# matteo-bastico/MI-Seg

Measured on AMD Instinct MI355X. Metric: 96^3 patches/sec fwd+bwd, C-Swin-UNETR fs=48 6-class, higher is better.
Workload: dtype bf16; 1 GPU; configs[1]: C-Swin-UNETR feature_size=48 heads=(3,6,12,24) instance_cond, 96^3 patch, 6 classes, batch 1 per GPU, fwd+bwd (+ gradient all-reduce at N>1); global_batch=1

## Files before the change

include/miseg_hip.h:

```cpp
#ifndef MISEG_HIP_H
#define MISEG_HIP_H
#include <stddef.h>
#include <stdint.h>

#ifdef __cplusplus
extern "C" {
#endif

typedef void* miseg_stream_t;

enum { MISEG_F32 = 0, MISEG_BF16 = 1 };
enum { MISEG_OK = 0, MISEG_E_BADARG = -1, MISEG_E_UNSUPPORTED = -2, MISEG_E_LAUNCH = -3 };
enum { MISEG_ACT_NONE = 0, MISEG_ACT_LEAKY = 1, MISEG_ACT_GELU = 2, MISEG_ACT_PRELU = 3 };
#define MISEG_MAX_STYLES 4

#define MISEG_ABI_VERSION 16
int miseg_abi_version(void);
const char* miseg_last_error(void);
int miseg_device_arch(char* buf, size_t n);

size_t miseg_instnorm_stat_bytes(int B, int C);
typedef struct {
  const void* x; int64_t ldx;
  int B, S, C, dtype;
// ... 205 lines not shown
  int wd, wh, ww, sd, sh, sw, tw;
  float scale;
  float drop_p; uint64_t drop_seed, drop_stream; const uint64_t* drop_step_dev;
} miseg_winattn_params;
int miseg_winattn_fwd(const miseg_winattn_params* p, miseg_stream_t stream);
int miseg_winattn_on_matrix_cores(const miseg_winattn_params* p);

typedef struct {
  miseg_winattn_params f;
  const void* dout; int64_t lddo;
  void* dqkv; int64_t lddq;
  float* dqkv_bias;
  float* dbias_table;
} miseg_winattn_bwd_params;
int miseg_winattn_bwd(const miseg_winattn_bwd_params* p, miseg_stream_t stream);

typedef struct { const void* a; int64_t lda; const void* b; int64_t ldb; void* y; int64_t ldy; int64_t rows; int C, dtype; } miseg_add_params;
int miseg_add(const miseg_add_params* p, miseg_stream_t stream);
typedef struct { uint32_t struct_size; const void* a; int64_t lda; const void* x; int64_t ldx; void* y; int64_t ldy; const float* coef; int B, S, C, dtype; } miseg_affine2_params;
int miseg_affine2(const miseg_affine2_params* p, miseg_stream_t stream);

typedef struct { const void* src; int64_t lds; int sdtype; void* dst; int64_t ldd; int ddtype; int64_t rows; int C; } miseg_copy2d_params;
int miseg_copy2d(const miseg_copy2d_params* p, miseg_stream_t stream);

typedef struct { const float* src; void* dst; int R, C, dtype, transpose; } miseg_cast_params;
int miseg_cast_matrix(const miseg_cast_params* p, miseg_stream_t stream);

typedef struct {
  const float* src; void* dst;
  int32_t R, C, transpose, inner, outer, tile0;
// ... 222 lines not shown
```

include/miseg_hip_debug.h:

```cpp
#ifndef MISEG_HIP_DEBUG_H
#define MISEG_HIP_DEBUG_H
#include "miseg_hip.h"
#ifdef __cplusplus
extern "C" {
#endif

int miseg_flag_wait(const uint64_t* flag_dev, const uint64_t* want_dev, uint64_t timeout_us, uint32_t* timed_out_dev, miseg_stream_t stream);
int miseg_streams_run_concurrently(miseg_stream_t a, miseg_stream_t b);
int miseg_debug_stamp(uint64_t* slot_dev, miseg_stream_t stream);

int miseg_prof_arm(int tag);
int miseg_prof_read(int* tags, float* ms, int max);

typedef void* miseg_graph_split_t;
typedef struct {
  int nodes, lanes, segments, crossing_edges, side_streams, main_lane_nodes;
  int streams_concurrent;
} miseg_graph_split_info;
int miseg_graph_split_create(void* hip_graph, miseg_stream_t launch_stream, int max_side_streams, miseg_graph_split_t* out,
                             miseg_graph_split_info* info );
int miseg_graph_split_launch(miseg_graph_split_t plan, miseg_stream_t stream);
void miseg_graph_split_destroy(miseg_graph_split_t plan);

int miseg_prof_available(void);

#ifdef __cplusplus
}
#endif
#endif
```

mi-seg_amd/csrc/attention.hip:

```cpp
#include "common.h"

namespace miseg {

struct WinGeom {
  int B, D, H, W, C, heads, hd;
  int wd, wh, ww, sd, sh, sw, tw;
  int Dp, Hp, Wp, nwd, nwh, nww, n;
  float scale;
};

__device__ __forceinline__ void token_info(const WinGeom& g, int win, int t, int& row, int& label, int& code) {
  int wi = win;
  const int wx = wi % g.nww; wi /= g.nww;
  const int wy = wi % g.nwh; wi /= g.nwh;
  const int wz = wi % g.nwd;
  const int b = wi / g.nwd;
  const int tz = t / (g.wh * g.ww), ty = (t / g.ww) % g.wh, tx = t % g.ww;
  const int pz = wz * g.wd + tz, py = wy * g.wh + ty, px = wx * g.ww + tx;
  int z = pz + g.sd; if (z >= g.Dp) z -= g.Dp;
  int y = py + g.sh; if (y >= g.Hp) y -= g.Hp;
  int x = px + g.sw; if (x >= g.Wp) x -= g.Wp;
  row = (z < g.D && y < g.H && x < g.W) ? ((b * g.D + z) * g.H + y) * g.W + x : -1;
  const int rz = g.sd ? (pz < g.Dp - g.wd ? 0 : (pz < g.Dp - g.sd ? 1 : 2)) : 0;
  const int ry = g.sh ? (py < g.Hp - g.wh ? 0 : (py < g.Hp - g.sh ? 1 : 2)) : 0;
// ... 337 lines not shown
  }
  return f;
}

__device__ __forceinline__ void att_load16v(const bf16* p, bool vec, float* dst) {
  if (vec) {
    const bf16x8 a = *reinterpret_cast<const bf16x8*>(p), b = *reinterpret_cast<const bf16x8*>(p + 8);
#pragma unroll
    for (int d = 0; d < 8; ++d) { dst[d] = to_f32(a[d]); dst[8 + d] = to_f32(b[d]); }
  } else {
#pragma unroll
    for (int d = 0; d < 16; ++d) dst[d] = to_f32(p[d]);
  }
}

__device__ __forceinline__ void att_unit(int heads, int& win, int& head) {
  const int nb = gridDim.x, xcd = blockIdx.x & 7, q = nb >> 3, r = nb & 7;
  const int unit = xcd * q + (xcd < r ? xcd : r) + (blockIdx.x >> 3);
  win = unit / heads;
  head = unit - win * heads;
}

template <bool MASK, int NW = 4, bool DROP = false>
__global__ void __launch_bounds__(NW * 64) winattn_fwd_mfma_kernel(const bf16* __restrict__ qkv, int64_t ldq, bf16* __restrict__ out, int64_t ldo,
                                                               const float* __restrict__ qkv_bias, const float* __restrict__ bias_table,
                                                               float* __restrict__ lse_out, WinGeom g, int tsize, bool vec, AttnDrop dr) {
  extern __shared__ __attribute__((aligned(16))) char smem[];
  bf16* Qs = reinterpret_cast<bf16*>(smem);
  bf16* Ks = Qs + ATT_NP * 16;
  bf16* Vt = Ks + ATT_NP * 16;
  int* kofs = reinterpret_cast<int*>(Vt + 16 * ATT_VT_LD);
  int* klab = kofs + ATT_NP;
  int* rowq = klab + ATT_NP;
// ... 156 lines not shown
#pragma unroll
    for (int d = 0; d < 8; ++d) { dst[d] = to_f32(a[d]); dst[8 + d] = to_f32(b[d]); }
  } else {
#pragma unroll
    for (int d = 0; d < 16; ++d) dst[d] = to_f32(p[d]);
  }
}

typedef unsigned pk2 __attribute__((ext_vector_type(2)));
__device__ __forceinline__ unsigned att_pk_bf16(float a, float b) {
  typedef float f32x2_ __attribute__((ext_vector_type(2)));
  typedef __bf16 bf16x2_ __attribute__((ext_vector_type(2)));
  return __builtin_bit_cast(unsigned, __builtin_convertvector(f32x2_{a, b}, bf16x2_));
}

template <bool MASK, bool DT , int NW = 4, bool DROP = false>
__global__ void __launch_bounds__(NW * 64, 2) winattn_bwd_mfma_kernel(const bf16* __restrict__ qkv, int64_t ldq, const bf16* __restrict__ out, int64_t ldo,
                                                                  const bf16* __restrict__ dout, int64_t lddo, bf16* __restrict__ dqkv, int64_t lddq,
                                                                  const float* __restrict__ qkv_bias, const float* __restrict__ bias_table,
                                                                  const float* __restrict__ lse_in, float* __restrict__ dqkv_bias,
                                                                  float* __restrict__ dbias_table, WinGeom g, int tsize, bool vec, AttnDrop dr) {
  extern __shared__ __attribute__((aligned(16))) char smem[];
  constexpr int NI = 24 / NW, NTHR = NW * 64;
  float* table = reinterpret_cast<float*>(smem);
  int* dtable = reinterpret_cast<int*>(table + ATT_TMAX);
  float* padb = reinterpret_cast<float*>(dtable + ATT_TMAX);
  unsigned* bound = reinterpret_cast<unsigned*>(padb + 48);
  char* dstile = reinterpret_cast<char*>(padb + 64);
  float* dqpart = reinterpret_cast<float*>(dstile + NW * 16 * ATT_DS_LD);
  int* qcode = reinterpret_cast<int*>(dqpart + 2 * NW * 256);
  int* qlabel = qcode + ATT_NP;
  int* rowq = qlabel + ATT_NP;
  float* nlse = reinterpret_cast<float*>(rowq + ATT_NP);
  float* ndelta = nlse + ATT_NP;
  bf16* Qs = reinterpret_cast<bf16*>(ndelta + ATT_NP);
  bf16* Gs = Qs + ATT_NP * 16;
  bf16* Ks = Gs + ATT_NP * 16;
  int win, head;
  att_unit(g.heads, win, head);
  const int tid = threadIdx.x;
  const int n = g.n, C = g.C, nt16 = (n + 15) / 16;
  if (tid < 52) padb[tid] = 0.f;
  __syncthreads();
  float mg2 = 0.f, mv2 = 0.f, mda = 0.f;
  for (int t = tid; t < nt16 * 16; t += NTHR) {
    int row = -1, label = 0, code = 0;
    float q[16], k[16], go[16];
    float dl = 0.f, ls = INFINITY, g2 = 0.f, v2 = 0.f;
#pragma unroll
    for (int d = 0; d < 16; ++d) q[d] = k[d] = go[d] = 0.f;
    if (t < n) {
      token_info(g, win, t, row, label, code);
      ls = lse_in[((int64_t)win * g.heads + head) * n + t];
      float v[16];
      if (row >= 0) {
        float o[16];
        att_load16(qkv + (int64_t)row * ldq + head * 16, vec, q);
        att_load16(qkv + (int64_t)row * ldq + C + head * 16, vec, k);
        att_load16(qkv + (int64_t)row * ldq + 2 * C + head * 16, vec, v);
        att_load16(dout + (int64_t)row * lddo + head * 16, vec, go);
        att_load16(out + (int64_t)row * ldo + head * 16, vec, o);
#pragma unroll
        for (int d = 0; d < 16; ++d) { dl = fmaf(go[d], o[d], dl); g2 = fmaf(go[d], go[d], g2); }
      } else {
#pragma unroll
        for (int d = 0; d < 16; ++d) {
          q[d] = qkv_bias ? qkv_bias[head * 16 + d] : 0.f;
          k[d] = qkv_bias ? qkv_bias[C + head * 16 + d] : 0.f;
          v[d] = qkv_bias ? qkv_bias[2 * C + head * 16 + d] : 0.f;
        }
      }
#pragma unroll
      for (int d = 0; d < 16; ++d) v2 = fmaf(v[d], v[d], v2);
    }
    mg2 = fmaxf(mg2, g2); mv2 = fmaxf(mv2, v2); mda = fmaxf(mda, fabsf(dl));
    const float qs = g.scale * ATT_LOG2E;
#pragma unroll
    for (int d = 0; d < 16; ++d) q[d] *= qs;
    att_store_row(Qs, t, q);
    att_store_row(Ks, t, k);
    att_store_row(Gs, t, go);
    qcode[t] = code * 4;
    qlabel[t] = label;
    rowq[t] = row;
    nlse[t] = -ls * ATT_LOG2E;
    ndelta[t] = -dl;
  }
#pragma unroll
  for (int o2 = 1; o2 < 64; o2 <<= 1) { mg2 = fmaxf(mg2, __shfl_xor(mg2, o2, 64)); mv2 = fmaxf(mv2, __shfl_xor(mv2, o2, 64)); mda = fmaxf(mda, __shfl_xor(mda, o2, 64)); }
  if ((tid & 63) == 0) { atomicMax(&bound[0], __float_as_uint(mg2)); atomicMax(&bound[1], __float_as_uint(mv2)); atomicMax(&bound[2], __float_as_uint(mda)); }
  for (int i = tid; i < tsize; i += NTHR) { table[i] = bias_table[(int64_t)i * g.heads + head] * ATT_LOG2E; dtable[i] = 0; }
  __syncthreads();
  const float bmax = sqrtf(__uint_as_float(bound[0]) * __uint_as_float(bound[1])) + __uint_as_float(bound[2]);
  const float fscale = bmax > 0.f ? 536870912.f / ((float)(n > 256 ? n : 256) * bmax) : 0.f;
  const int lane = tid & 63, wave = __builtin_amdgcn_readfirstlane(tid >> 6), fi = lane & 15, kg = lane >> 4;
  const int tb = 2 * g.tw - 1;
  const int centre = ((g.tw - 1) * tb + (g.tw - 1)) * tb + (g.tw - 1);
  constexpr float MASKV = -100.f * ATT_LOG2E;

  s16x4 kfB[NI], vfB[NI], kA[NI];
  f32x4 dvt[NI], dkt[NI];
  int ck[NI], lk[NI];
  const char* tkb[NI];
  bool kval = true;
  int itail = -1;
#pragma unroll
  for (int i = 0; i < NI; ++i) {
    const int kt = wave + NW * i;
    dvt[i] = dkt[i] = f32x4{0.f, 0.f, 0.f, 0.f};
    kfB[i] = vfB[i] = kA[i] = s16x4{0, 0, 0, 0};
    ck[i] = lk[i] = 0;
    tkb[i] = reinterpret_cast<const char*>(table);
    if (kt < nt16) {
      const int ki = kt * 16 + fi;
      kfB[i] = att_ld4(Ks, ki, kg);
      kA[i] = att_tr_rows(Ks, kt * 16, fi, kg);
      ck[i] = qcode[ki] - 4 * centre;
      tkb[i] = reinterpret_cast<const char*>(table) - ck[i];
      lk[i] = qlabel[ki];
      float v[4] = {0.f, 0.f, 0.f, 0.f};
      if (ki < n) {
        const int row = rowq[ki];
        if (row >= 0) {
          const bf16x4 t4 = *reinterpret_cast<const bf16x4*>(qkv + (int64_t)row * ldq + 2 * C + head * 16 + 4 * kg);
#pragma unroll
          for (int e = 0; e < 4; ++e) v[e] = to_f32(t4[e]);
        } else if (qkv_bias) {
#pragma unroll
          for (int e = 0; e < 4; ++e) v[e] = qkv_bias[2 * C + head * 16 + 4 * kg + e];
        }
      }
      vfB[i] = __builtin_bit_cast(s16x4, bf16x4{(bf16)v[0], (bf16)v[1], (bf16)v[2], (bf16)v[3]});
      if (kt == nt16 - 1 && (n & 15)) { itail = i; kval = ki < n; }
    }
  }
  const uint64_t dk0 = DROP ? dropout_step_key(dr.key, dr.step_dev) : 0ull;
  const int dcg = (n + 3) / 4;
  const int64_t dbase = ((int64_t)win * g.heads + head) * n;
  char* mytile = dstile + wave * 16 * ATT_DS_LD;
  char* const ds_w = mytile + fi * ATT_DS_LD + kg * 8;
  const char* const ds_r = mytile + (4 * kg + (fi >> 2)) * ATT_DS_LD + (fi & 3) * 8;

  f32x4 padq = f32x4{0.f, 0.f, 0.f, 0.f};
  for (int qt = 0; qt < nt16; ++qt) {
    const int q0 = qt * 16;
    const int4 qc4 = *reinterpret_cast<const int4*>(qcode + q0 + 4 * kg);
    const int qc[4] = {qc4.x, qc4.y, qc4.z, qc4.w};
    int ql[4] = {0, 0, 0, 0};
    if (MASK) {
      const int4 ql4 = *reinterpret_cast<const int4*>(qlabel + q0 + 4 * kg);
      ql[0] = ql4.x; ql[1] = ql4.y; ql[2] = ql4.z; ql[3] = ql4.w;
    }
    const f32x4 nl4 = *reinterpret_cast<const f32x4*>(nlse + q0 + 4 * kg);
    const f32x4 nd4 = *reinterpret_cast<const f32x4*>(ndelta + q0 + 4 * kg);
    const s16x4 qfA = att_ld4(Qs, q0 + fi, kg);
    const s16x4 gfA = att_ld4(Gs, q0 + fi, kg);
    const s16x4 qtA = att_tr_rows(Qs, q0, fi, kg);
    const s16x4 gtA = att_tr_rows(Gs, q0, fi, kg);
    f32x4 dq = f32x4{0.f, 0.f, 0.f, 0.f};
#pragma unroll
    for (int i = 0; i < NI; ++i) {
      if (wave + NW * i < nt16) {
        const f32x4 sacc = __builtin_amdgcn_mfma_f32_16x16x16bf16_1k(qfA, kfB[i], nl4, 0, 0, 0);
        const f32x4 pacc = __builtin_amdgcn_mfma_f32_16x16x16bf16_1k(gfA, vfB[i], DROP ? f32x4{0.f, 0.f, 0.f, 0.f} : nd4, 0, 0, 0);
        float pv[4], dsv[4], tbv[4];
        int bidx[4];
#pragma unroll
        for (int e = 0; e < 4; ++e) {
          bidx[e] = qc[e] - ck[i];
          tbv[e] = *reinterpret_cast<const float*>(tkb[i] + qc[e]);
        }
#pragma unroll
        for (int e = 0; e < 4; ++e) {
          float sc = sacc[e] + tbv[e];
          if (MASK) sc += (ql[e] != lk[i]) ? MASKV : 0.f;
          pv[e] = __builtin_amdgcn_exp2f(sc);
        }
        if (i == itail) {
#pragma unroll
          for (int e = 0; e < 4; ++e) pv[e] = kval ? pv[e] : 0.f;
        }
        float pm[4];
        if (DROP) {
          const int ki = (wave + NW * i) * 16 + fi;
#pragma unroll
          for (int e = 0; e < 4; ++e) {
            const uint64_t hh = dropout_group_hash(dk0, dbase + q0 + 4 * kg + e, dcg, ki);
            pm[e] = dropout_keeps(hh, ki, dr.thresh) ? pv[e] * dr.scale : 0.f;
            dsv[e] = fmaf(pm[e], pacc[e], pv[e] * nd4[e]);
          }
        } else {
#pragma unroll
          for (int e = 0; e < 4; ++e) { pm[e] = pv[e]; dsv[e] = pv[e] * pacc[e]; }
        }
        const pk2 pbp = pk2{att_pk_bf16(pm[0], pm[1]), att_pk_bf16(pm[2], pm[3])};
        const pk2 dbp = pk2{att_pk_bf16(dsv[0], dsv[1]), att_pk_bf16(dsv[2], dsv[3])};
        const s16x4 pb = __builtin_bit_cast(s16x4, pbp), db = __builtin_bit_cast(s16x4, dbp);
        const bf16x4 db4 = __builtin_bit_cast(bf16x4, dbp);
        dvt[i] = __builtin_amdgcn_mfma_f32_16x16x16bf16_1k(gtA, pb, dvt[i], 0, 0, 0);
        dkt[i] = __builtin_amdgcn_mfma_f32_16x16x16bf16_1k(qtA, db, dkt[i], 0, 0, 0);
        *reinterpret_cast<bf16x4*>(ds_w) = db4;
        __builtin_amdgcn_fence(__ATOMIC_RELEASE, "wavefront");
        __builtin_amdgcn_wave_barrier();
        __builtin_amdgcn_fence(__ATOMIC_ACQUIRE, "wavefront");
        const s16x4 dsT = att_tr4(ds_r);
        dq = __builtin_amdgcn_mfma_f32_16x16x16bf16_1k(kA[i], dsT, dq, 0, 0, 0);
        __builtin_amdgcn_wave_barrier();
        if (DT) {
#pragma unroll
          for (int e = 0; e < 4; ++e)
            atomicAdd(reinterpret_cast<int*>(reinterpret_cast<char*>(dtable) + bidx[e]), __float_as_int(fmaf(dsv[e], fscale, 12582912.f)) - 0x4B400000);
        }
      }
    }
    float* part = dqpart + (qt & 1) * (NW * 256);
    *reinterpret_cast<f32x4*>(part + (wave * 16 + fi) * 16 + 4 * kg) = dq;
    __syncthreads();
    if (wave == (qt & (NW - 1))) {
      const int ql_ = lane >> 2, d4 = lane & 3, t = q0 + ql_;
      f32x4 sum = *reinterpret_cast<const f32x4*>(part + ql_ * 16 + 4 * d4);
#pragma unroll
      for (int w = 1; w < NW; ++w) sum += *reinterpret_cast<const f32x4*>(part + (w * 16 + ql_) * 16 + 4 * d4);
      if (t < n) {
        const int row = rowq[t];
        if (row >= 0) {
          *reinterpret_cast<bf16x4*>(dqkv + (int64_t)row * lddq + head * 16 + 4 * d4) =
              bf16x4{(bf16)(sum[0] * g.scale), (bf16)(sum[1] * g.scale), (bf16)(sum[2] * g.scale), (bf16)(sum[3] * g.scale)};
        } else if (dqkv_bias) {
          padq += sum;
        }
      }
    }
  }
  if (dqkv_bias) {
#pragma unroll
    for (int o2 = 4; o2 < 64; o2 <<= 1)
#pragma unroll
      for (int e = 0; e < 4; ++e) padq[e] += __shfl_xor(padq[e], o2, 64);
    if (lane < 4) {
#pragma unroll
      for (int e = 0; e < 4; ++e)
        if (padq[e] != 0.f) atomicAdd(&padb[4 * lane + e], padq[e] * g.scale);
    }
  }
  constexpr float LN2 = 0.6931471805599453f;
  f32x4 padk = f32x4{0.f, 0.f, 0.f, 0.f}, padv = f32x4{0.f, 0.f, 0.f, 0.f};
#pragma unroll
  for (int i = 0; i < NI; ++i) {
    const int ki = (wave + NW * i) * 16 + fi;
    if (wave + NW * i < nt16 && ki < n) {
      const int row = rowq[ki];
      if (row >= 0) {
        bf16* pk = dqkv + (int64_t)row * lddq + C + head * 16 + 4 * kg;
        *reinterpret_cast<bf16x4*>(pk) = bf16x4{(bf16)(dkt[i][0] * LN2), (bf16)(dkt[i][1] * LN2), (bf16)(dkt[i][2] * LN2), (bf16)(dkt[i][3] * LN2)};
        *reinterpret_cast<bf16x4*>(pk + C) = bf16x4{(bf16)dvt[i][0], (bf16)dvt[i][1], (bf16)dvt[i][2], (bf16)dvt[i][3]};
      } else if (dqkv_bias) {
        padk += dkt[i];
        padv += dvt[i];
      }
    }
  }
  if (dqkv_bias) {
#pragma unroll
    for (int o2 = 1; o2 < 16; o2 <<= 1)
#pragma unroll
      for (int e = 0; e < 4; ++e) { padk[e] += __shfl_xor(padk[e], o2, 64); padv[e] += __shfl_xor(padv[e], o2, 64); }
    if (fi == 0) {
#pragma unroll
      for (int e = 0; e < 4; ++e) {
        if (padk[e] != 0.f) atomicAdd(&padb[16 + 4 * kg + e], padk[e] * LN2);
        if (padv[e] != 0.f) atomicAdd(&padb[32 + 4 * kg + e], padv[e]);
      }
    }
  }
  __syncthreads();
  if (dbias_table)
    for (int i = tid; i < tsize; i += NTHR) {
      const int v = dtable[i];
      if (v != 0) atomicAdd(dbias_table + (int64_t)i * g.heads + head, (float)v / fscale);
    }
  if (dqkv_bias && tid < 48) {
    const float v = padb[tid];
    if (v != 0.f) atomicAdd(dqkv_bias + (tid >> 4) * C + head * 16 + (tid & 15), v);
  }
}

static size_t attn_mfma_bwd_smem(int tsize, int nw = 4) {
  (void)tsize;
  return (size_t)3 * ATT_NP * 32 + (size_t)5 * ATT_NP * 4 + (size_t)2 * nw * 256 * 4 + (size_t)nw * 16 * ATT_DS_LD + 64 * 4 + (size_t)2 * ATT_TMAX * 4;
}

static size_t attn_mfma_fwd_smem(int tsize) {
  return (size_t)(2 * ATT_NP * 16 + 16 * ATT_VT_LD) * 2 + (size_t)3 * ATT_NP * 4 + (size_t)tsize * 4;
}

int global_attn_fwd(const miseg_winattn_params* p, const AttnDrop& dr, hipStream_t s, int* rc);
int global_attn_bwd(const miseg_winattn_bwd_params* p, const AttnDrop& dr, hipStream_t s, int* rc);
bool global_attn_takes(const miseg_winattn_params* p);

// ... 79 lines not shown
#undef FWD_MFMA_D
    MISEG_LAUNCH_CHECK("winattn_fwd_mfma");
    return MISEG_OK;
  }
  return dispatch_dtype(p->dtype, [&](auto* tag) -> int {
    typedef typename std::remove_pointer<decltype(tag)>::type T;
    HD_SWITCH(g.hd / 4, {
      MISEG_SET_SMEM((winattn_fwd_kernel<T, HD4>), sh);
      winattn_fwd_kernel<T, HD4><<<grid, threads, sh, s>>>((const T*)p->qkv, p->ldq, (T*)p->out, p->ldo, p->qkv_bias, p->bias_table, p->lse, g, tsize, dr);
    });
    MISEG_LAUNCH_CHECK("winattn_fwd");
    return MISEG_OK;
  });
}

extern "C" int miseg_winattn_bwd(const miseg_winattn_bwd_params* p, miseg_stream_t s_) {
  hipStream_t s = (hipStream_t)s_;
  MISEG_REQUIRE(p && p->dout && p->dqkv, MISEG_E_BADARG, "winattn_bwd: null pointer");
  WinGeom g;
  int rc = make_geom(&p->f, &g);
  if (rc) return rc;
  MISEG_REQUIRE(p->f.drop_p >= 0.f && p->f.drop_p < 1.f, MISEG_E_BADARG, "winattn_bwd: drop_p = %f must lie in [0, 1)", (double)p->f.drop_p);
  const AttnDrop dr = attn_drop_args(&p->f);
  if (global_attn_bwd(p, dr, s, &rc)) return rc;
  const int tb = 2 * g.tw - 1, tsize = p->f.bias_table ? tb * tb * tb : 0;
  const size_t sh = attn_smem_bytes(g.n, g.hd, tsize, true);
  MISEG_REQUIRE(sh <= 160 * 1024, MISEG_E_UNSUPPORTED, "winattn_bwd: %zu bytes of LDS needed", sh);
  dim3 grid(g.B * g.nwd * g.nwh * g.nww, g.heads);
  const int threads = cdiv(g.n, 64) * 64;
  if (p->f.dtype == MISEG_BF16 && g.hd == 16 && g.n <= ATT_NP && p->f.bias_table && tsize <= ATT_TMAX && ((uintptr_t)p->dqkv % 8 == 0) && p->lddq % 4 == 0 &&
      ((uintptr_t)p->f.qkv % 8 == 0) && p->f.ldq % 4 == 0) {
    const bool vec = p->f.ldq % 8 == 0 && p->f.ldo % 8 == 0 && p->lddo % 8 == 0 && (uintptr_t)p->f.qkv % 16 == 0 && (uintptr_t)p->f.out % 16 == 0 &&
                     (uintptr_t)p->dout % 16 == 0;
    const bool wide = true;
    const size_t shm = attn_mfma_bwd_smem(tsize, wide ? 8 : 4);
#define BWD_MFMA_X(M, D, NWV, X)                                                                                                                            \
  MISEG_SET_SMEM((winattn_bwd_mfma_kernel<M, D, NWV, X>), shm);                              \
  winattn_bwd_mfma_kernel<M, D, NWV, X><<<grid.x * grid.y, NWV * 64, shm, s>>>((const bf16*)p->f.qkv, p->f.ldq, (const bf16*)p->f.out, p->f.ldo, (const bf16*)p->dout,    \
                                                                    p->lddo, (bf16*)p->dqkv, p->lddq, p->f.qkv_bias, p->f.bias_table, p->f.lse, p->dqkv_bias, \
                                                                    p->dbias_table, g, tsize, vec, dr)
#define BWD_MFMA(M, D, NWV) do { if (dr.thresh) { BWD_MFMA_X(M, D, NWV, true); } else { BWD_MFMA_X(M, D, NWV, false); } } while (0)
#define BWD_MFMA_W(M, D) do { if (wide) { BWD_MFMA(M, D, 8); } else { BWD_MFMA(M, D, 4); } } while (0)
    const bool masked = (g.sd | g.sh | g.sw) != 0;
    if (p->dbias_table) { if (masked) BWD_MFMA_W(true, true); else BWD_MFMA_W(false, true); }
    else { if (masked) BWD_MFMA_W(true, false); else BWD_MFMA_W(false, false); }
#undef BWD_MFMA_W
#undef BWD_MFMA
#undef BWD_MFMA_X
    MISEG_LAUNCH_CHECK("winattn_bwd_mfma");
    return MISEG_OK;
  }
  return dispatch_dtype(p->f.dtype, [&](auto* tag) -> int {
    typedef typename std::remove_pointer<decltype(tag)>::type T;
    HD_SWITCH(g.hd / 4, {
      MISEG_SET_SMEM((winattn_bwd_kernel<T, HD4>), sh);
      winattn_bwd_kernel<T, HD4><<<grid, threads, sh, s>>>((const T*)p->f.qkv, p->f.ldq, (const T*)p->f.out, p->f.ldo, (const T*)p->dout, p->lddo, (T*)p->dqkv, p->lddq,
                                                           p->f.qkv_bias, p->f.bias_table, p->f.lse, p->dqkv_bias, p->dbias_table ? p->dbias_table : nullptr, g,
                                                           tsize, dr);
    });
    MISEG_LAUNCH_CHECK("winattn_bwd");
// ... 4 lines not shown
```

mi-seg_amd/hip/lib.py:

```python
import ctypes as C
import os

HERE = os.path.dirname(os.path.abspath(__file__))
LIB_PATH = os.environ.get("MISEG_HIP_LIB") or os.path.join(os.path.dirname(HERE), "csrc", "libmiseg_hip.so")

F32, BF16 = 0, 1
ACT_NONE, ACT_LEAKY, ACT_GELU, ACT_PRELU = 0, 1, 2, 3
MAX_STYLES = 4

vp, i64, i32, f32 = C.c_void_p, C.c_int64, C.c_int, C.c_float
fp4 = vp * MAX_STYLES


class _S(C.Structure):
    pass


ABI_VERSION = 16
C_NAMES = {}


def _struct(name, fields, cname=None):
    t = type(name, (C.Structure,), {"_fields_": fields})
    C_NAMES[t] = cname
# ... 184 lines not shown
    "miseg_gemm_tn_stream_group_target": (i32, []),
    "miseg_colsum_batch": (i32, [vp, i32, i32, vp]),
    "miseg_conv3_fwd_plan": (i32, [C.POINTER(Conv3), C.POINTER(Conv3Plan)]),
    "miseg_conv3_fwd": (i32, [C.POINTER(Conv3), vp]),
    "miseg_pack_conv3_elems": (C.c_size_t, [i32, i32, i32, i32]),
    "miseg_pack_conv3_tiles": (i32, [i32, i32, i32]),
    "miseg_pack_conv3_weight": (i32, [C.POINTER(PackConv3), vp]),
    "miseg_pack_conv3_batch": (i32, [vp, i32, i32, i32, vp, vp, vp]),
    "miseg_conv3_wgrad_plan": (i32, [C.POINTER(Conv3Wgrad), C.POINTER(Conv3WgradPlan)]),
    "miseg_conv3_wgrad": (i32, [C.POINTER(Conv3Wgrad), vp]),
    "miseg_conv3_wgrad_group_workspace_bytes": (C.c_size_t, [C.POINTER(Conv3Wgrad), i32]),
    "miseg_conv3_wgrad_group": (i32, [C.POINTER(Conv3Wgrad), i32, vp, vp]),
    "miseg_winattn_fwd": (i32, [C.POINTER(Winattn), vp]),
    "miseg_winattn_on_matrix_cores": (i32, [vp]),
    "miseg_winattn_bwd": (i32, [C.POINTER(WinattnBwd), vp]),
    "miseg_add": (i32, [C.POINTER(Add), vp]),
    "miseg_affine2": (i32, [C.POINTER(Affine2), vp]),
    "miseg_instnorm_bwd_reduce": (i32, [C.POINTER(InstnormBwd), vp]),
    "miseg_copy2d": (i32, [C.POINTER(Copy2d), vp]),
    "miseg_cast_matrix": (i32, [C.POINTER(Cast), vp]),
    "miseg_gelu_fwd": (i32, [C.POINTER(GeluFwd), vp]),
    "miseg_gelu_bwd": (i32, [C.POINTER(GeluBwd), vp]),
    "miseg_space_to_channel": (i32, [C.POINTER(S2C), vp]),
    "miseg_channel_to_space": (i32, [C.POINTER(S2C), vp]),
    "miseg_patch_embed_fwd": (i32, [C.POINTER(PatchEmbed), vp]),
    "miseg_patch_embed_bwd_workspace_bytes": (C.c_size_t, [C.POINTER(PatchEmbedBwd)]),
    "miseg_patch_embed_bwd": (i32, [C.POINTER(PatchEmbedBwd), vp]),
    "miseg_conv3_thin_fwd": (i32, [C.POINTER(Conv3Thin), vp]),
    "miseg_conv3_thin_wgrad_workspace_bytes": (C.c_size_t, [C.POINTER(Conv3ThinWgrad)]),
    "miseg_conv3_thin_wgrad": (i32, [C.POINTER(Conv3ThinWgrad), vp]),
# ... 32 lines not shown
    "miseg_counter_copy": (i32, [vp, vp, vp]),
    "miseg_abi_struct_size": (C.c_size_t, [C.c_char_p]),
    "miseg_device_check": (i32, [i32]),
    "miseg_source_digest": (C.c_char_p, []),
}
DEBUG_PROTOS = {
    "miseg_debug_stamp": (i32, [vp, vp]),
    "miseg_prof_arm": (i32, [i32]),
    "miseg_prof_read": (i32, [vp, vp, i32]),
    "miseg_prof_available": (i32, []),
    "miseg_flag_wait": (i32, [vp, vp, C.c_uint64, vp, vp]),
    "miseg_streams_run_concurrently": (i32, [vp, vp]),
    "miseg_graph_split_create": (i32, [vp, vp, i32, C.POINTER(vp), vp]),
    "miseg_graph_split_launch": (i32, [vp, vp]),
    "miseg_graph_split_destroy": (None, [vp]),
}
DEBUG_STRUCTS = {"miseg_graph_split_info"}
PROF_LIB_PATH = os.path.join(os.path.dirname(LIB_PATH), "libmiseg_hip_prof.so")

_lib = None


class MisegHipError(RuntimeError):
    pass


def source_digest():
    try:
        from ..csrc import build as _b
        return _b.source_digest()
# ... 60 lines not shown
```

Before: 168.0 patches/s.

## Split window-attention backward into dQ and dKV role workgroups for small grids

When the number of (window, head) units is below the CU count, the backward attention kernel splits each unit into several dQ workgroups (over query tiles) and dKV workgroups (over key tiles), picked by a small cost model. Each role skips the loads and MFMAs it does not need. The aim is to fill the GPU on deep Swin stages that have few windows. In exchange, S and dP are recomputed in both roles and staging work is duplicated across workgroups. Debug hooks allow forcing the split and listing the tiles each part covers.

Result: no change. 168.2 patches/s (median of 6 runs) (+0.1%).

```diff
diff --git a/include/miseg_hip.h b/include/miseg_hip.h
--- a/include/miseg_hip.h
+++ b/include/miseg_hip.h
@@ -243,6 +243,7 @@
   float* dbias_table;
 } miseg_winattn_bwd_params;
 int miseg_winattn_bwd(const miseg_winattn_bwd_params* p, miseg_stream_t stream);
+int miseg_winattn_bwd_plan(const miseg_winattn_bwd_params* p, int* sq, int* sk);
 
 typedef struct { const void* a; int64_t lda; const void* b; int64_t ldb; void* y; int64_t ldy; int64_t rows; int C, dtype; } miseg_add_params;
 int miseg_add(const miseg_add_params* p, miseg_stream_t stream);
diff --git a/include/miseg_hip_debug.h b/include/miseg_hip_debug.h
--- a/include/miseg_hip_debug.h
+++ b/include/miseg_hip_debug.h
@@ -22,6 +22,9 @@
 int miseg_graph_split_launch(miseg_graph_split_t plan, miseg_stream_t stream);
 void miseg_graph_split_destroy(miseg_graph_split_t plan);
 
+int miseg_debug_winattn_split(int sq, int sk);
+int miseg_debug_winattn_split_tiles(int nt16, int sq, int sk, int part, int* tiles, int max);
+
 int miseg_prof_available(void);
 
 #ifdef __cplusplus
diff --git a/mi-seg_amd/csrc/attention.hip b/mi-seg_amd/csrc/attention.hip
--- a/mi-seg_amd/csrc/attention.hip
+++ b/mi-seg_amd/csrc/attention.hip
@@ -1,4 +1,6 @@
 #include "common.h"
+#include <atomic>
+#include "miseg_hip_debug.h"
 
 namespace miseg {
 
@@ -375,9 +377,13 @@
   }
 }
 
+__device__ __forceinline__ int att_slot() {
+  const int nb = gridDim.x, xcd = blockIdx.x & 7, q = nb >> 3, r = nb & 7;
+  return xcd * q + (xcd < r ? xcd : r) + (blockIdx.x >> 3);
+}
+
 __device__ __forceinline__ void att_unit(int heads, int& win, int& head) {
-  const int nb = gridDim.x, xcd = blockIdx.x & 7, q = nb >> 3, r = nb & 7;
-  const int unit = xcd * q + (xcd < r ? xcd : r) + (blockIdx.x >> 3);
+  const int unit = att_slot();
   win = unit / heads;
   head = unit - win * heads;
 }
@@ -564,13 +570,19 @@
   return __builtin_bit_cast(unsigned, __builtin_convertvector(f32x2_{a, b}, bf16x2_));
 }
 
-template <bool MASK, bool DT , int NW = 4, bool DROP = false>
-__global__ void __launch_bounds__(NW * 64, 2) winattn_bwd_mfma_kernel(const bf16* __restrict__ qkv, int64_t ldq, const bf16* __restrict__ out, int64_t ldo,
-                                                                  const bf16* __restrict__ dout, int64_t lddo, bf16* __restrict__ dqkv, int64_t lddq,
-                                                                  const float* __restrict__ qkv_bias, const float* __restrict__ bias_table,
-                                                                  const float* __restrict__ lse_in, float* __restrict__ dqkv_bias,
-                                                                  float* __restrict__ dbias_table, WinGeom g, int tsize, bool vec, AttnDrop dr) {
-  extern __shared__ __attribute__((aligned(16))) char smem[];
+enum { ATT_ALL = 0, ATT_DQ = 1, ATT_DKV = 2 };
+
+__host__ __device__ inline int att_split_q0(int nt16, int sq, int p) { return (int)((int64_t)p * nt16 / sq); }
+__host__ __device__ inline int att_split_kt(int sk, int p, int nw, int wave, int i) { return p + sk * (wave + nw * i); }
+
+template <int ROLE, bool MASK, bool DT , int NW, bool DROP>
+__device__ __forceinline__ void winattn_bwd_mfma_body(char* smem, int win, int head, int part, int nparts, const bf16* __restrict__ qkv, int64_t ldq,
+                                                      const bf16* __restrict__ out, int64_t ldo, const bf16* __restrict__ dout, int64_t lddo,
+                                                      bf16* __restrict__ dqkv, int64_t lddq, const float* __restrict__ qkv_bias,
+                                                      const float* __restrict__ bias_table, const float* __restrict__ lse_in,
+                                                      float* __restrict__ dqkv_bias, float* __restrict__ dbias_table, const WinGeom& g, int tsize, bool vec,
+                                                      const AttnDrop& dr) {
+  constexpr bool DO_Q = ROLE != ATT_DKV, DO_KV = ROLE != ATT_DQ;
   constexpr int NI = 24 / NW, NTHR = NW * 64;
   float* table = reinterpret_cast<float*>(smem);
   int* dtable = reinterpret_cast<int*>(table + ATT_TMAX);
@@ -586,10 +598,9 @@
   bf16* Qs = reinterpret_cast<bf16*>(ndelta + ATT_NP);
   bf16* Gs = Qs + ATT_NP * 16;
   bf16* Ks = Gs + ATT_NP * 16;
-  int win, head;
-  att_unit(g.heads, win, head);
   const int tid = threadIdx.x;
   const int n = g.n, C = g.C, nt16 = (n + 15) / 16;
+  const int qt_lo = ROLE == ATT_DQ ? att_split_q0(nt16, nparts, part) : 0, qt_hi = ROLE == ATT_DQ ? att_split_q0(nt16, nparts, part + 1) : nt16;
   if (tid < 52) padb[tid] = 0.f;
   __syncthreads();
   float mg2 = 0.f, mv2 = 0.f, mda = 0.f;
@@ -597,27 +608,36 @@
     int row = -1, label = 0, code = 0;
     float q[16], k[16], go[16];
     float dl = 0.f, ls = INFINITY, g2 = 0.f, v2 = 0.f;
+    const bool myq = ROLE != ATT_DQ || (t >= qt_lo * 16 && t < qt_hi * 16);
 #pragma unroll
     for (int d = 0; d < 16; ++d) q[d] = k[d] = go[d] = 0.f;
     if (t < n) {
       token_info(g, win, t, row, label, code);
-      ls = lse_in[((int64_t)win * g.heads + head) * n + t];
+      if (myq) ls = lse_in[((int64_t)win * g.heads + head) * n + t];
       float v[16];
+#pragma unroll
+      for (int d = 0; d < 16; ++d) v[d] = 0.f;
       if (row >= 0) {
-        float o[16];
-        att_load16(qkv + (int64_t)row * ldq + head * 16, vec, q);
-        att_load16(qkv + (int64_t)row * ldq + C + head * 16, vec, k);
-        att_load16(qkv + (int64_t)row * ldq + 2 * C + head * 16, vec, v);
-        att_load16(dout + (int64_t)row * lddo + head * 16, vec, go);
-        att_load16(out + (int64_t)row * ldo + head * 16, vec, o);
-#pragma unroll
-        for (int d = 0; d < 16; ++d) { dl = fmaf(go[d], o[d], dl); g2 = fmaf(go[d], go[d], g2); }
+        if (myq) {
+          float o[16];
+          att_load16(qkv + (int64_t)row * ldq + head * 16, vec, q);
+          att_load16(dout + (int64_t)row * lddo + head * 16, vec, go);
+          att_load16(out + (int64_t)row * ldo + head * 16, vec, o);
+#pragma unroll
+          for (int d = 0; d < 16; ++d) { dl = fmaf(go[d], o[d], dl); g2 = fmaf(go[d], go[d], g2); }
+        }
+        if (DO_Q) {
+          att_load16(qkv + (int64_t)row * ldq + C + head * 16, vec, k);
+          att_load16(qkv + (int64_t)row * ldq + 2 * C + head * 16, vec, v);
+        }
       } else {
 #pragma unroll
         for (int d = 0; d < 16; ++d) {
           q[d] = qkv_bias ? qkv_bias[head * 16 + d] : 0.f;
-          k[d] = qkv_bias ? qkv_bias[C + head * 16 + d] : 0.f;
-          v[d] = qkv_bias ? qkv_bias[2 * C + head * 16 + d] : 0.f;
+          if (DO_Q) {
+            k[d] = qkv_bias ? qkv_bias[C + head * 16 + d] : 0.f;
+            v[d] = qkv_bias ? qkv_bias[2 * C + head * 16 + d] : 0.f;
+          }
         }
       }
 #pragma unroll
@@ -627,19 +647,23 @@
     const float qs = g.scale * ATT_LOG2E;
 #pragma unroll
     for (int d = 0; d < 16; ++d) q[d] *= qs;
-    att_store_row(Qs, t, q);
-    att_store_row(Ks, t, k);
-    att_store_row(Gs, t, go);
+    if (myq) {
+      att_store_row(Qs, t, q);
+      att_store_row(Gs, t, go);
+      nlse[t] = -ls * ATT_LOG2E;
+      ndelta[t] = -dl;
+    }
+    if (DO_Q) att_store_row(Ks, t, k);
     qcode[t] = code * 4;
     qlabel[t] = label;
     rowq[t] = row;
-    nlse[t] = -ls * ATT_LOG2E;
-    ndelta[t] = -dl;
-  }
-#pragma unroll
-  for (int o2 = 1; o2 < 64; o2 <<= 1) { mg2 = fmaxf(mg2, __shfl_xor(mg2, o2, 64)); mv2 = fmaxf(mv2, __shfl_xor(mv2, o2, 64)); mda = fmaxf(mda, __shfl_xor(mda, o2, 64)); }
-  if ((tid & 63) == 0) { atomicMax(&bound[0], __float_as_uint(mg2)); atomicMax(&bound[1], __float_as_uint(mv2)); atomicMax(&bound[2], __float_as_uint(mda)); }
-  for (int i = tid; i < tsize; i += NTHR) { table[i] = bias_table[(int64_t)i * g.heads + head] * ATT_LOG2E; dtable[i] = 0; }
+  }
+  if (DO_Q) {
+#pragma unroll
+    for (int o2 = 1; o2 < 64; o2 <<= 1) { mg2 = fmaxf(mg2, __shfl_xor(mg2, o2, 64)); mv2 = fmaxf(mv2, __shfl_xor(mv2, o2, 64)); mda = fmaxf(mda, __shfl_xor(mda, o2, 64)); }
+    if ((tid & 63) == 0) { atomicMax(&bound[0], __float_as_uint(mg2)); atomicMax(&bound[1], __float_as_uint(mv2)); atomicMax(&bound[2], __float_as_uint(mda)); }
+  }
+  for (int i = tid; i < tsize; i += NTHR) { table[i] = bias_table[(int64_t)i * g.heads + head] * ATT_LOG2E; if (DO_Q) dtable[i] = 0; }
   __syncthreads();
   const float bmax = sqrtf(__uint_as_float(bound[0]) * __uint_as_float(bound[1])) + __uint_as_float(bound[2]);
   const float fscale = bmax > 0.f ? 536870912.f / ((float)(n > 256 ? n : 256) * bmax) : 0.f;
@@ -654,33 +678,45 @@
   const char* tkb[NI];
   bool kval = true;
   int itail = -1;
+  const int ksk = ROLE == ATT_DKV ? nparts : 1, kp = ROLE == ATT_DKV ? part : 0;
 #pragma unroll
   for (int i = 0; i < NI; ++i) {
-    const int kt = wave + NW * i;
+    const int kt = att_split_kt(ksk, kp, NW, wave, i);
     dvt[i] = dkt[i] = f32x4{0.f, 0.f, 0.f, 0.f};
     kfB[i] = vfB[i] = kA[i] = s16x4{0, 0, 0, 0};
     ck[i] = lk[i] = 0;
     tkb[i] = reinterpret_cast<const char*>(table);
     if (kt < nt16) {
       const int ki = kt * 16 + fi;
-      kfB[i] = att_ld4(Ks, ki, kg);
-      kA[i] = att_tr_rows(Ks, kt * 16, fi, kg);
+      if (DO_Q) {
+        kfB[i] = att_ld4(Ks, ki, kg);
+        kA[i] = att_tr_rows(Ks, kt * 16, fi, kg);
+      }
       ck[i] = qcode[ki] - 4 * centre;
       tkb[i] = reinterpret_cast<const char*>(table) - ck[i];
       lk[i] = qlabel[ki];
-      float v[4] = {0.f, 0.f, 0.f, 0.f};
+      float v[4] = {0.f, 0.f, 0.f, 0.f}, k4[4] = {0.f, 0.f, 0.f, 0.f};
       if (ki < n) {
         const int row = rowq[ki];
         if (row >= 0) {
           const bf16x4 t4 = *reinterpret_cast<const bf16x4*>(qkv + (int64_t)row * ldq + 2 * C + head * 16 + 4 * kg);
 #pragma unroll
           for (int e = 0; e < 4; ++e) v[e] = to_f32(t4[e]);
+          if (!DO_Q) {
+            const bf16x4 u4 = *reinterpret_cast<const bf16x4*>(qkv + (int64_t)row * ldq + C + head * 16 + 4 * kg);
+#pragma unroll
+            for (int e = 0; e < 4; ++e) k4[e] = to_f32(u4[e]);
+          }
         } else if (qkv_bias) {
 #pragma unroll
-          for (int e = 0; e < 4; ++e) v[e] = qkv_bias[2 * C + head * 16 + 4 * kg + e];
+          for (int e = 0; e < 4; ++e) {
+            v[e] = qkv_bias[2 * C + head * 16 + 4 * kg + e];
+            if (!DO_Q) k4[e] = qkv_bias[C + head * 16 + 4 * kg + e];
+          }
         }
       }
       vfB[i] = __builtin_bit_cast(s16x4, bf16x4{(bf16)v[0], (bf16)v[1], (bf16)v[2], (bf16)v[3]});
+      if (!DO_Q) kfB[i] = __builtin_bit_cast(s16x4, bf16x4{(bf16)k4[0], (bf16)k4[1], (bf16)k4[2], (bf16)k4[3]});
       if (kt == nt16 - 1 && (n & 15)) { itail = i; kval = ki < n; }
     }
   }
@@ -692,7 +728,7 @@
   const char* const ds_r = mytile + (4 * kg + (fi >> 2)) * ATT_DS_LD + (fi & 3) * 8;
 
   f32x4 padq = f32x4{0.f, 0.f, 0.f, 0.f};
-  for (int qt = 0; qt < nt16; ++qt) {
+  for (int qt = qt_lo; qt < qt_hi; ++qt) {
     const int q0 = qt * 16;
     const int4 qc4 = *reinterpret_cast<const int4*>(qcode + q0 + 4 * kg);
     const int qc[4] = {qc4.x, qc4.y, qc4.z, qc4.w};
@@ -705,12 +741,15 @@
     const f32x4 nd4 = *reinterpret_cast<const f32x4*>(ndelta + q0 + 4 * kg);
     const s16x4 qfA = att_ld4(Qs, q0 + fi, kg);
     const s16x4 gfA = att_ld4(Gs, q0 + fi, kg);
-    const s16x4 qtA = att_tr_rows(Qs, q0, fi, kg);
-    const s16x4 gtA = att_tr_rows(Gs, q0, fi, kg);
+    s16x4 qtA = s16x4{0, 0, 0, 0}, gtA = s16x4{0, 0, 0, 0};
+    if (DO_KV) {
+      qtA = att_tr_rows(Qs, q0, fi, kg);
+      gtA = att_tr_rows(Gs, q0, fi, kg);
+    }
     f32x4 dq = f32x4{0.f, 0.f, 0.f, 0.f};
 #pragma unroll
     for (int i = 0; i < NI; ++i) {
-      if (wave + NW * i < nt16) {
+      if (att_split_kt(ksk, kp, NW, wave, i) < nt16) {
         const f32x4 sacc = __builtin_amdgcn_mfma_f32_16x16x16bf16_1k(qfA, kfB[i], nl4, 0, 0, 0);
         const f32x4 pacc = __builtin_amdgcn_mfma_f32_16x16x16bf16_1k(gfA, vfB[i], DROP ? f32x4{0.f, 0.f, 0.f, 0.f} : nd4, 0, 0, 0);
         float pv[4], dsv[4], tbv[4];
@@ -732,7 +771,7 @@
         }
         float pm[4];
         if (DROP) {
-          const int ki = (wave + NW * i) * 16 + fi;
+          const int ki = att_split_kt(ksk, kp, NW, wave, i) * 16 + fi;
 #pragma unroll
           for (int e = 0; e < 4; ++e) {
             const uint64_t hh = dropout_group_hash(dk0, dbase + q0 + 4 * kg + e, dcg, ki);
@@ -747,42 +786,48 @@
         const pk2 dbp = pk2{att_pk_bf16(dsv[0], dsv[1]), att_pk_bf16(dsv[2], dsv[3])};
         const s16x4 pb = __builtin_bit_cast(s16x4, pbp), db = __builtin_bit_cast(s16x4, dbp);
         const bf16x4 db4 = __builtin_bit_cast(bf16x4, dbp);
-        dvt[i] = __builtin_amdgcn_mfma_f32_16x16x16bf16_1k(gtA, pb, dvt[i], 0, 0, 0);
-        dkt[i] = __builtin_amdgcn_mfma_f32_16x16x16bf16_1k(qtA, db, dkt[i], 0, 0, 0);
-        *reinterpret_cast<bf16x4*>(ds_w) = db4;
-        __builtin_amdgcn_fence(__ATOMIC_RELEASE, "wavefront");
-        __builtin_amdgcn_wave_barrier();
-        __builtin_amdgcn_fence(__ATOMIC_ACQUIRE, "wavefront");
-        const s16x4 dsT = att_tr4(ds_r);
-        dq = __builtin_amdgcn_mfma_f32_16x16x16bf16_1k(kA[i], dsT, dq, 0, 0, 0);
-        __builtin_amdgcn_wave_barrier();
-        if (DT) {
-#pragma unroll
-          for (int e = 0; e < 4; ++e)
-            atomicAdd(reinterpret_cast<int*>(reinterpret_cast<char*>(dtable) + bidx[e]), __float_as_int(fmaf(dsv[e], fscale, 12582912.f)) - 0x4B400000);
-        }
-      }
-    }
-    float* part = dqpart + (qt & 1) * (NW * 256);
-    *reinterpret_cast<f32x4*>(part + (wave * 16 + fi) * 16 + 4 * kg) = dq;
-    __syncthreads();
-    if (wave == (qt & (NW - 1))) {
-      const int ql_ = lane >> 2, d4 = lane & 3, t = q0 + ql_;
-      f32x4 sum = *reinterpret_cast<const f32x4*>(part + ql_ * 16 + 4 * d4);
-#pragma unroll
-      for (int w = 1; w < NW; ++w) sum += *reinterpret_cast<const f32x4*>(part + (w * 16 + ql_) * 16 + 4 * d4);
-      if (t < n) {
-        const int row = rowq[t];
-        if (row >= 0) {
-          *reinterpret_cast<bf16x4*>(dqkv + (int64_t)row * lddq + head * 16 + 4 * d4) =
-              bf16x4{(bf16)(sum[0] * g.scale), (bf16)(sum[1] * g.scale), (bf16)(sum[2] * g.scale), (bf16)(sum[3] * g.scale)};
-        } else if (dqkv_bias) {
-          padq += sum;
-        }
-      }
-    }
-  }
-  if (dqkv_bias) {
+        if (DO_KV) {
+          dvt[i] = __builtin_amdgcn_mfma_f32_16x16x16bf16_1k(gtA, pb, dvt[i], 0, 0, 0);
+          dkt[i] = __builtin_amdgcn_mfma_f32_16x16x16bf16_1k(qtA, db, dkt[i], 0, 0, 0);
+        }
+        if (DO_Q) {
+          *reinterpret_cast<bf16x4*>(ds_w) = db4;
+          __builtin_amdgcn_fence(__ATOMIC_RELEASE, "wavefront");
+          __builtin_amdgcn_wave_barrier();
+          __builtin_amdgcn_fence(__ATOMIC_ACQUIRE, "wavefront");
+          const s16x4 dsT = att_tr4(ds_r);
+          dq = __builtin_amdgcn_mfma_f32_16x16x16bf16_1k(kA[i], dsT, dq, 0, 0, 0);
+          __builtin_amdgcn_wave_barrier();
+          if (DT) {
+#pragma unroll
+            for (int e = 0; e < 4; ++e)
+              atomicAdd(reinterpret_cast<int*>(reinterpret_cast<char*>(dtable) + bidx[e]), __float_as_int(fmaf(dsv[e], fscale, 12582912.f)) - 0x4B400000);
+          }
+        }
+      }
+    }
+    if (DO_Q) {
+      float* part_dq = dqpart + (qt & 1) * (NW * 256);
+      *reinterpret_cast<f32x4*>(part_dq + (wave * 16 + fi) * 16 + 4 * kg) = dq;
+      __syncthreads();
+      if (wave == (qt & (NW - 1))) {
+        const int ql_ = lane >> 2, d4 = lane & 3, t = q0 + ql_;
+        f32x4 sum = *reinterpret_cast<const f32x4*>(part_dq + ql_ * 16 + 4 * d4);
+#pragma unroll
+        for (int w = 1; w < NW; ++w) sum += *reinterpret_cast<const f32x4*>(part_dq + (w * 16 + ql_) * 16 + 4 * d4);
+        if (t < n) {
+          const int row = rowq[t];
+          if (row >= 0) {
+            *reinterpret_cast<bf16x4*>(dqkv + (int64_t)row * lddq + head * 16 + 4 * d4) =
+                bf16x4{(bf16)(sum[0] * g.scale), (bf16)(sum[1] * g.scale), (bf16)(sum[2] * g.scale), (bf16)(sum[3] * g.scale)};
+          } else if (dqkv_bias) {
+            padq += sum;
+          }
+        }
+      }
+    }
+  }
+  if (DO_Q && dqkv_bias) {
 #pragma unroll
     for (int o2 = 4; o2 < 64; o2 <<= 1)
 #pragma unroll
@@ -797,8 +842,8 @@
   f32x4 padk = f32x4{0.f, 0.f, 0.f, 0.f}, padv = f32x4{0.f, 0.f, 0.f, 0.f};
 #pragma unroll
   for (int i = 0; i < NI; ++i) {
-    const int ki = (wave + NW * i) * 16 + fi;
-    if (wave + NW * i < nt16 && ki < n) {
+    const int kt = att_split_kt(ksk, kp, NW, wave, i), ki = kt * 16 + fi;
+    if (DO_KV && kt < nt16 && ki < n) {
       const int row = rowq[ki];
       if (row >= 0) {
         bf16* pk = dqkv + (int64_t)row * lddq + C + head * 16 + 4 * kg;
@@ -810,7 +855,7 @@
       }
     }
   }
-  if (dqkv_bias) {
+  if (DO_KV && dqkv_bias) {
 #pragma unroll
     for (int o2 = 1; o2 < 16; o2 <<= 1)
 #pragma unroll
@@ -824,7 +869,7 @@
     }
   }
   __syncthreads();
-  if (dbias_table)
+  if (DO_Q && dbias_table)
     for (int i = tid; i < tsize; i += NTHR) {
       const int v = dtable[i];
       if (v != 0) atomicAdd(dbias_table + (int64_t)i * g.heads + head, (float)v / fscale);
@@ -833,6 +878,36 @@
     const float v = padb[tid];
     if (v != 0.f) atomicAdd(dqkv_bias + (tid >> 4) * C + head * 16 + (tid & 15), v);
   }
+}
+
+template <bool MASK, bool DT, int NW = 4, bool DROP = false>
+__global__ void __launch_bounds__(NW * 64, 2) winattn_bwd_mfma_kernel(const bf16* __restrict__ qkv, int64_t ldq, const bf16* __restrict__ out, int64_t ldo,
+                                                                  const bf16* __restrict__ dout, int64_t lddo, bf16* __restrict__ dqkv, int64_t lddq,
+                                                                  const float* __restrict__ qkv_bias, const float* __restrict__ bias_table,
+                                                                  const float* __restrict__ lse_in, float* __restrict__ dqkv_bias,
+                                                                  float* __restrict__ dbias_table, WinGeom g, int tsize, bool vec, AttnDrop dr) {
+  extern __shared__ __attribute__((aligned(16))) char smem[];
+  int win, head;
+  att_unit(g.heads, win, head);
+  winattn_bwd_mfma_body<ATT_ALL, MASK, DT, NW, DROP>(smem, win, head, 0, 1, qkv, ldq, out, ldo, dout, lddo, dqkv, lddq, qkv_bias, bias_table, lse_in, dqkv_bias,
+                                                     dbias_table, g, tsize, vec, dr);
+}
+
+template <bool MASK, bool DT, int NW, bool DROP>
+__global__ void __launch_bounds__(NW * 64, 2) winattn_bwd_roles_kernel(const bf16* __restrict__ qkv, int64_t ldq, const bf16* __restrict__ out, int64_t ldo,
+                                                                   const bf16* __restrict__ dout, int64_t lddo, bf16* __restrict__ dqkv, int64_t lddq,
+                                                                   const float* __restrict__ qkv_bias, const float* __restrict__ bias_table,
+                                                                   const float* __restrict__ lse_in, float* __restrict__ dqkv_bias,
+                                                                   float* __restrict__ dbias_table, WinGeom g, int tsize, bool vec, AttnDrop dr, int sq, int sk) {
+  extern __shared__ __attribute__((aligned(16))) char smem[];
+  const int slot = att_slot(), np = sq + sk, unit = slot / np, part = slot - unit * np;
+  const int win = unit / g.heads, head = unit - win * g.heads;
+  if (part < sq)
+    winattn_bwd_mfma_body<ATT_DQ, MASK, DT, NW, DROP>(smem, win, head, part, sq, qkv, ldq, out, ldo, dout, lddo, dqkv, lddq, qkv_bias, bias_table, lse_in,
+                                                      dqkv_bias, dbias_table, g, tsize, vec, dr);
+  else
+    winattn_bwd_mfma_body<ATT_DKV, MASK, false, NW, DROP>(smem, win, head, part - sq, sk, qkv, ldq, out, ldo, dout, lddo, dqkv, lddq, qkv_bias, bias_table,
+                                                          lse_in, dqkv_bias, dbias_table, g, tsize, vec, dr);
 }
 
 static size_t attn_mfma_bwd_smem(int tsize, int nw = 4) {
@@ -942,6 +1017,66 @@
   });
 }
 
+static constexpr int ATT_BWD_NW = 8;
+static constexpr int ATT_CUS = 256;
+static constexpr int ATT_STEP_DQ = 7, ATT_STEP_DKV = 2;
+static int att_bwd_chain(int qtiles, int ktiles_per_wave, int step) { return qtiles * (step + ktiles_per_wave); }
+
+static void att_bwd_plan(int units, int nt16, int* sq, int* sk) {
+  *sq = *sk = 1;
+  if (units >= ATT_CUS) return;
+  const int budget = 2 * ATT_CUS / units;
+  long best = -1;
+  for (int k = 1; k <= nt16 && k < budget; ++k)
+    for (int q = 1; q <= nt16 && q + k <= budget; ++q) {
+      if (q + k < 3) continue;
+      const int cq = att_bwd_chain(cdiv(nt16, q), cdiv(nt16, ATT_BWD_NW), ATT_STEP_DQ), ck = att_bwd_chain(nt16, cdiv(cdiv(nt16, k), ATT_BWD_NW), ATT_STEP_DKV);
+      const long cost = (long)(cq > ck ? cq : ck) * 1024 + (q + k);
+      if (best < 0 || cost < best) { best = cost; *sq = q; *sk = k; }
+    }
+}
+
+static std::atomic<int> g_bwd_split_sq{0}, g_bwd_split_sk{0};
+
+static bool bwd_shape(const miseg_winattn_params* f, int* units, int* n) {
+  if (!(f->B > 0 && f->D > 0 && f->H > 0 && f->W > 0 && f->C > 0 && f->heads > 0 && f->wd > 0 && f->wh > 0 && f->ww > 0)) return false;
+  *units = f->B * cdiv(f->D, f->wd) * cdiv(f->H, f->wh) * cdiv(f->W, f->ww) * f->heads;
+  *n = f->wd * f->wh * f->ww;
+  return true;
+}
+
+extern "C" int miseg_winattn_bwd_plan(const miseg_winattn_bwd_params* p, int* sq, int* sk) {
+  MISEG_REQUIRE(p && sq && sk, MISEG_E_BADARG, "winattn_bwd_plan: null pointer");
+  int units, n;
+  MISEG_REQUIRE(bwd_shape(&p->f, &units, &n), MISEG_E_BADARG, "winattn_bwd_plan: bad shape");
+  *sq = *sk = 1;
+  if (p->f.dtype == MISEG_BF16 && p->f.C == 16 * p->f.heads && n <= ATT_NP) att_bwd_plan(units, (n + 15) / 16, sq, sk);
+  return MISEG_OK;
+}
+
+extern "C" int miseg_debug_winattn_split(int sq, int sk) {
+  MISEG_REQUIRE((sq == 0 && sk == 0) || (sq > 0 && sk > 0), MISEG_E_BADARG, "debug_winattn_split: (%d, %d): both 0 (the plan decides) or both positive", sq, sk);
+  g_bwd_split_sq = sq;
+  g_bwd_split_sk = sk;
+  return MISEG_OK;
+}
+
+extern "C" int miseg_debug_winattn_split_tiles(int nt16, int sq, int sk, int part, int* tiles, int max) {
+  MISEG_REQUIRE(nt16 > 0 && sq > 0 && sk > 0 && part >= 0 && part < sq + sk && tiles && max >= 0, MISEG_E_BADARG, "debug_winattn_split_tiles: bad argument");
+  int c = 0;
+  if (part < sq) {
+    for (int t = att_split_q0(nt16, sq, part); t < att_split_q0(nt16, sq, part + 1); ++t, ++c)
+      if (c < max) tiles[c] = t;
+  } else {
+    for (int w = 0; w < ATT_BWD_NW; ++w)
+      for (int i = 0; i < 24 / ATT_BWD_NW; ++i) {
+        const int kt = att_split_kt(sk, part - sq, ATT_BWD_NW, w, i);
+        if (kt < nt16) { if (c < max) tiles[c] = kt; ++c; }
+      }
+  }
+  return c;
+}
+
 extern "C" int miseg_winattn_bwd(const miseg_winattn_bwd_params* p, miseg_stream_t s_) {
   hipStream_t s = (hipStream_t)s_;
   MISEG_REQUIRE(p && p->dout && p->dqkv, MISEG_E_BADARG, "winattn_bwd: null pointer");
@@ -969,9 +1104,26 @@
                                                                     p->dbias_table, g, tsize, vec, dr)
 #define BWD_MFMA(M, D, NWV) do { if (dr.thresh) { BWD_MFMA_X(M, D, NWV, true); } else { BWD_MFMA_X(M, D, NWV, false); } } while (0)
 #define BWD_MFMA_W(M, D) do { if (wide) { BWD_MFMA(M, D, 8); } else { BWD_MFMA(M, D, 4); } } while (0)
+#define BWD_ROLES_X(M, D, X)                                                                                                                                 \
+  MISEG_SET_SMEM((winattn_bwd_roles_kernel<M, D, ATT_BWD_NW, X>), shm);                                                                                      \
+  winattn_bwd_roles_kernel<M, D, ATT_BWD_NW, X><<<grid.x * grid.y * (sq + sk), ATT_BWD_NW * 64, shm, s>>>(                                                    \
+      (const bf16*)p->f.qkv, p->f.ldq, (const bf16*)p->f.out, p->f.ldo, (const bf16*)p->dout, p->lddo, (bf16*)p->dqkv, p->lddq, p->f.qkv_bias, p->f.bias_table, \
+      p->f.lse, p->dqkv_bias, p->dbias_table, g, tsize, vec, dr, sq, sk)
+#define BWD_ROLES(M, D) do { if (dr.thresh) { BWD_ROLES_X(M, D, true); } else { BWD_ROLES_X(M, D, false); } } while (0)
     const bool masked = (g.sd | g.sh | g.sw) != 0;
-    if (p->dbias_table) { if (masked) BWD_MFMA_W(true, true); else BWD_MFMA_W(false, true); }
+    const int nt16 = (g.n + 15) / 16;
+    int sq = g_bwd_split_sq, sk = g_bwd_split_sk;
+    if (sq <= 0 || sk <= 0) att_bwd_plan((int)(grid.x * grid.y), nt16, &sq, &sk);
+    sq = sq < nt16 ? sq : nt16;
+    sk = sk < nt16 ? sk : nt16;
+    if (sq * sk > 1) {
+      static_assert(ATT_BWD_NW == 8, "the role form is the 8-wave workgroup");
+      if (p->dbias_table) { if (masked) BWD_ROLES(true, true); else BWD_ROLES(false, true); }
+      else { if (masked) BWD_ROLES(true, false); else BWD_ROLES(false, false); }
+    } else if (p->dbias_table) { if (masked) BWD_MFMA_W(true, true); else BWD_MFMA_W(false, true); }
     else { if (masked) BWD_MFMA_W(true, false); else BWD_MFMA_W(false, false); }
+#undef BWD_ROLES
+#undef BWD_ROLES_X
 #undef BWD_MFMA_W
 #undef BWD_MFMA
 #undef BWD_MFMA_X
diff --git a/mi-seg_amd/hip/lib.py b/mi-seg_amd/hip/lib.py
--- a/mi-seg_amd/hip/lib.py
+++ b/mi-seg_amd/hip/lib.py
@@ -222,6 +222,7 @@
     "miseg_winattn_fwd": (i32, [C.POINTER(Winattn), vp]),
     "miseg_winattn_on_matrix_cores": (i32, [vp]),
     "miseg_winattn_bwd": (i32, [C.POINTER(WinattnBwd), vp]),
+    "miseg_winattn_bwd_plan": (i32, [C.POINTER(WinattnBwd), C.POINTER(i32), C.POINTER(i32)]),
     "miseg_add": (i32, [C.POINTER(Add), vp]),
     "miseg_affine2": (i32, [C.POINTER(Affine2), vp]),
     "miseg_instnorm_bwd_reduce": (i32, [C.POINTER(InstnormBwd), vp]),
@@ -284,6 +285,8 @@
     "miseg_graph_split_create": (i32, [vp, vp, i32, C.POINTER(vp), vp]),
     "miseg_graph_split_launch": (i32, [vp, vp]),
     "miseg_graph_split_destroy": (None, [vp]),
+    "miseg_debug_winattn_split": (i32, [i32, i32]),
+    "miseg_debug_winattn_split_tiles": (i32, [i32, i32, i32, i32, C.POINTER(i32), i32]),
 }
 DEBUG_STRUCTS = {"miseg_graph_split_info"}
 PROF_LIB_PATH = os.path.join(os.path.dirname(LIB_PATH), "libmiseg_hip_prof.so")
```
